# cs2mosa/Heterogeneous-MOE-for-Diffusion-models

Measured on AMD Instinct MI355X. Metric: denoise-steps/sec (fwd+bwd) on 4x32x32 latents, higher is better.
Workload: dtype bf16

## Files before the change

heterogeneous-moe-for-diffusion-models_amd/csrc/bwd6.hip:

```cpp
#include "common.h"
#include "conv_args.h"
#include "conv6_common.h"
#include "hdmoe.h"
#include "conv6_body.h"
#include "conv7_body.h"
#include "wgrad6_body.h"
#include "wgrad7_body.h"
#include "wgrad8_body.h"
#include "conv6s_body.h"

namespace {

template <int MT, int NT, int TWS, int OT>
__global__ __launch_bounds__(512) void bwd6_kernel(C6Args c, W6Args a3, W6Args a5, int G6, int ibs, int obs) {
  const int b = blockIdx.x;
  if (b < G6) { conv6_body<MT, NT>(c, b, G6); return; }
  int r = b - G6;
  const int bx = r % ibs; r /= ibs;
  const int by = r % obs;
  const int z = r / obs;
  if (z < a3.chunks) wgrad6_body<3, TWS, OT, false>(a3, bx, by, z);
  else wgrad6_body<5, TWS, OT, false>(a5, bx, by, z - a3.chunks);
}

template <int MT, int NT, int TWS, int OT>
void launch_bwd6(const C6Plan& cp, const W6DualPlan& wp, hipStream_t stream) {
  static unsigned long long attr = 0;
  if (hdmoe_first_on_device(attr)) { (void)hipFuncSetAttribute((const void*)bwd6_kernel<MT, NT, TWS, OT>, hipFuncAttributeMaxDynamicSharedMemorySize, 160 * 1024); }
  const size_t lds = cp.lds > wp.lds ? cp.lds : wp.lds;
  const unsigned grid = cp.G + (unsigned)(wp.ibs * wp.obs * (wp.c[0].chunks + wp.c[1].chunks));
  hipLaunchKernelGGL((bwd6_kernel<MT, NT, TWS, OT>), dim3(grid), dim3(512), lds, stream, cp.a, wp.c[0], wp.c[1], (int)cp.G, wp.ibs, wp.obs);
}

template <int CO, int KMASK, int TWS, int OT>
__global__ __launch_bounds__(512) void bwd7_kernel(C7Args c, W6Args a3, W6Args a5, int G7, int ibs, int obs) {
  const int b = blockIdx.x;
  if (b < G7) { conv7_body<CO, KMASK, TWS == 4>(c, b, G7); return; }
  int r = b - G7;
  if (TWS == 5 && OT == 0) {
    const int nbx3 = a3.Cin / (32 * a3.icw), nby3 = a3.Cout / (32 * a3.ocw), n3 = nbx3 * nby3 * a3.chunks;
    if (r < n3) {
      const int bx = r % nbx3; r /= nbx3;
      const int by = r % nby3, z = r / nby3, pairs = a3.icw * a3.ocw;
      if (pairs == 0) wgrad7_body<3>(a3, bx, by, z);
      else if (pairs == 4) wgrad8_body3<4, 8>(a3, bx, by, z);
      else if (pairs == 2) wgrad8_body3<2, 8>(a3, bx, by, z);
      else wgrad8_body3<2, 16>(a3, bx, by, z);
      return;
    }
    r -= n3;
    const int bx = r % ibs; r /= ibs;
    wgrad7_body<5>(a5, bx, r % obs, r / obs);
  } else if (OT > 0) {
    const int bx = r % ibs; r /= ibs;
    const int by = r % obs;
    const int z = r / obs;
    if (z < a3.chunks) wgrad6_body<3, TWS, OT == 0 ? 1 : OT, false>(a3, bx, by, z);
    else wgrad6_body<5, TWS, OT == 0 ? 1 : OT, false>(a5, bx, by, z - a3.chunks);
  }
}

template <int CO, int KMASK, int TWS, int OT>
void launch_bwd7(const C7Plan& cp, const W6DualPlan& wp, hipStream_t stream) {
  static unsigned long long attr = 0;
  if (hdmoe_first_on_device(attr)) { (void)hipFuncSetAttribute((const void*)bwd7_kernel<CO, KMASK, TWS, OT>, hipFuncAttributeMaxDynamicSharedMemorySize, 160 * 1024); }
  const size_t lds = cp.lds > wp.lds ? cp.lds : wp.lds;
  const int obs = OT == 0 ? wp.c[0].Cout / 32 : wp.obs;
  unsigned nw = (unsigned)(wp.ibs * obs * (wp.c[0].chunks + wp.c[1].chunks));
  if (OT == 0) nw = (unsigned)((wp.c[0].Cin / (32 * wp.c[0].icw)) * (wp.c[0].Cout / (32 * wp.c[0].ocw)) * wp.c[0].chunks + wp.ibs * obs * wp.c[1].chunks);
  hipLaunchKernelGGL((bwd7_kernel<CO, KMASK, TWS, OT>), dim3(cp.G + nw), dim3(512), lds, stream, cp.a, wp.c[0], wp.c[1], (int)cp.G, wp.ibs, obs);
}

template <int NT, int TWS, int OT>
__global__ __launch_bounds__(512) void bwd6s_kernel(C6SArgs c, W6Args a3, int G6, int ibs, int obs) {
  const int b = blockIdx.x;
  if (b < G6) { conv6s_body<NT>(c, b, G6); return; }
  int r = b - G6;
  const int bx = r % ibs; r /= ibs;
  wgrad6_body<3, TWS, OT, true>(a3, bx, r % obs, r / obs);
}
template <int NT, int TWS, int OT>
void launch_bwd6s(const C6SPlan& cp, const W6DualPlan& wp, hipStream_t stream) {
  static unsigned long long attr = 0;
  if (hdmoe_first_on_device(attr)) { (void)hipFuncSetAttribute((const void*)bwd6s_kernel<NT, TWS, OT>, hipFuncAttributeMaxDynamicSharedMemorySize, 160 * 1024); }
  const size_t lds = cp.lds > wp.lds ? cp.lds : wp.lds;
  const unsigned grid = cp.G + (unsigned)(wp.ibs * wp.obs * wp.c[0].chunks);
  hipLaunchKernelGGL((bwd6s_kernel<NT, TWS, OT>), dim3(grid), dim3(512), lds, stream, cp.sa, wp.c[0], (int)cp.G, wp.ibs, wp.obs);
}

}

extern "C" {

int hdmoe_conv_bwd6s(const void* x, const void* dy, const void* wd, void* dx, float* const* G, const int* seg, int ngroups, long wd_stride,
                     long wd_plane, int N, int H, int W, int Cin, int Cout, const int* kh, const int* kw, const int* pt, const int* pl,
                     float alpha, void* ws, long ws_bytes, const float* in_scale, const float* in_shift, int in_relu, int hi_only, hipStream_t stream) {
  if (!dx || !wd || ngroups < 1 || ngroups > HDMOE_MAX_GROUPS || Cout % 16) return 1;
  W6DualPlan wp;
  if (wgrad6_plan_split(x, dy, G, seg, ngroups, N, H, W, Cin, Cout, kh, kw, pt, pl, ws, ws_bytes, wp)) return 1;
  if ((in_scale == nullptr) != (in_shift == nullptr) || (in_scale && (ngroups != 1 || seg))) return HDMOE_EINVAL;
  wp.c[0].in_scale = in_scale; wp.c[0].in_shift = in_shift; wp.c[0].in_relu = in_relu;
  wp.c[0].hi_only = hi_only ? 1 : 0;
  const ConvArgs c = conv_dgrad_args(dy, wd, dx, seg, ngroups, wd_stride, N, H, W, Cin, Cout, kh, kw, pt, pl, alpha);
  C6SPlan cp;
  if (conv6s_plan(c, wd_plane, nullptr, cp)) return 1;
  cp.sa.nprod = hi_only ? 1 : 3;
  hdmoe_count_selection(HDMOE_SEL_BWD6S);
  conv_pick<2, 1>(cp.NT, [&](auto Nt) { conv_pick<5, 4>(wp.TWS, [&](auto Tws) { conv_pick<2, 1>(wp.OT, [&](auto Ot) {
    launch_bwd6s<decltype(Nt)::value, decltype(Tws)::value, decltype(Ot)::value>(cp, wp, stream);
  }); }); });
  return hdmoe_launch_status();
}

int hdmoe_conv_bwd6(const void* x, const void* dy, const void* wd, void* dx, float* const* G, const int* seg, int ngroups, long wd_stride,
                    int N, int H, int W, int Cin, int Cout, const int* kh, const int* kw, const int* pt, const int* pl, float alpha,
                    void* ws, long ws_bytes, int dtype, hipStream_t stream) {
  if (dtype != HDMOE_BF16 || !dx || !wd || ngroups < 1 || ngroups > HDMOE_MAX_GROUPS || Cout % 16) return 1;
  W6DualPlan wp;
  if (wgrad6_plan_dual(x, dy, G, seg, ngroups, N, H, W, Cin, Cout, kh, kw, pt, pl, ws, ws_bytes, dtype, wp)) return 1;
  const ConvArgs c = conv_dgrad_args(dy, wd, dx, seg, ngroups, wd_stride, N, H, W, Cin, Cout, kh, kw, pt, pl, alpha);
  {
    C7Plan cp7;
    if (!conv7_plan(c, dtype, cp7) && cp7.kmask == 3 && (cp7.w16 != 0) == (wp.TWS == 4)) {
      if (wp.TWS == 5) {
        hdmoe_count_selection(HDMOE_SEL_BWD7_32);
        if (wp.c[0].chunks) {
          hdmoe_count_selection(HDMOE_SEL_BWD7_32_WGRAD8);
          hdmoe_count_selection(wp.c[0].icw == 2 ? (wp.c[0].ocw == 2 ? HDMOE_SEL_WGRAD8_C22 : HDMOE_SEL_WGRAD8_C21)
                                                 : (wp.c[0].ocw == 2 ? HDMOE_SEL_WGRAD8_C12 : HDMOE_SEL_WGRAD8_C11));
        }
        if (wp.c[1].chunks) hdmoe_count_selection(HDMOE_SEL_BWD7_32_WGRAD7);
      } else {
        hdmoe_count_selection(wp.OT == 2 ? HDMOE_SEL_BWD7_16_OT2 : HDMOE_SEL_BWD7_16_OT1);
      }
      conv_pick<2, 1>(cp7.CO, [&](auto Co) {
        if (wp.TWS == 5) launch_bwd7<decltype(Co)::value, 3, 5, 0>(cp7, wp, stream);
        else conv_pick<2, 1>(wp.OT, [&](auto Ot) { launch_bwd7<decltype(Co)::value, 3, 4, decltype(Ot)::value>(cp7, wp, stream); });
      });
      return hdmoe_launch_status();
    }
  }
  C6Plan cp;
  if (conv6_plan(c, dtype, cp)) return 1;
  hdmoe_count_selection(HDMOE_SEL_BWD6);
  conv_pick<2, 1>(cp.MT, [&](auto M) { conv_pick<2, 1>(cp.NT, [&](auto Nt) { conv_pick<5, 4>(wp.TWS, [&](auto Tws) { conv_pick<2, 1>(wp.OT, [&](auto Ot) {
    launch_bwd6<decltype(M)::value, decltype(Nt)::value, decltype(Tws)::value, decltype(Ot)::value>(cp, wp, stream);
  }); }); }); });
  return hdmoe_launch_status();
}

}
```

heterogeneous-moe-for-diffusion-models_amd/csrc/wgrad8_body.h:

```cpp
#pragma once
#include "common.h"
#include "wgrad6_body.h"

namespace {

DEVI bool w8_slot(const W6Args& a, const int zslot, int& n0, int& n1) {
  int gi = 0, chunk = zslot, row0 = 0, units = 0;
  for (; gi < a.ngr; ++gi) {
    const int g = a.groups[gi];
    row0 = a.seg ? __builtin_amdgcn_readfirstlane(a.seg[g]) : 0;
    units = ((a.seg ? __builtin_amdgcn_readfirstlane(a.seg[g + 1]) : a.N) - row0) * a.tpi;
    const int nch = (units + a.upw - 1) / a.upw;
    if (chunk < nch) break;
    chunk -= nch;
  }
  if (gi == a.ngr) return false;
  const int t0 = chunk * a.upw, t1 = min(units, t0 + a.upw);
  n0 = row0 + t0 / 4; n1 = row0 + (t1 + 3) / 4;
  return true;
}

template <int NACC, typename TapOf, typename Store>
DEVI void w8_reduce(unsigned char* lds, const f32x16 (&acc)[NACC], const int NGR, const int wave, const int lane, const int tid, TapOf tap_of, Store store) {
  float* red = reinterpret_cast<float*>(lds);
  const int NP = 8 / NGR;
#pragma unroll
  for (int j0 = 0; j0 < NACC; j0 += 4) {
    const int nr = NACC - j0 < 4 ? NACC - j0 : 4;
    asm volatile("s_waitcnt lgkmcnt(0)\n\ts_barrier" ::: "memory");
#pragma unroll
    for (int jj = 0; jj < 4; ++jj)
      if (jj < nr) {
#pragma unroll
        for (int reg = 0; reg < 16; ++reg) red[((wave * 4 + jj) * 16 + reg) * 64 + lane] = acc[j0 + jj][reg];
      }
    asm volatile("s_waitcnt lgkmcnt(0)\n\ts_barrier" ::: "memory");
    const int ntask = NGR * nr * 256;
    for (int task = tid; task < ntask; task += 512) {
      const int e4 = task & 255, gj = task >> 8, jj = gj % nr, g = gj / nr;
      f32x4 s = (f32x4)(0.f);
      for (int k = 0; k < NP; ++k) s += *reinterpret_cast<const f32x4*>(red + (((g + NGR * k) * 4 + jj) * 1024 + e4 * 4));
      const int el = e4 * 4, reg = el >> 6, ln = el & 63;
      store(g, tap_of(g, j0 + jj), acc_row(reg, ln), ln & 31, s);
    }
  }
}

template <int RPW, int RU>
DEVI void wgrad8_body3(const W6Args& a, const int bx, const int by, const int zslot) {
#if __HIP_DEVICE_COMPILE__
  constexpr int Q = 2;
  constexpr int XROWS = RU + 2, XROWB = 35 * 64, XB = XROWS * XROWB + 3 * 64, DYB = RU * 2048, UPI = 32 / RU;
  extern __shared__ __attribute__((aligned(1024))) unsigned char lds[];
  const int tid = threadIdx.x, lane = tid & 63;
  const int wave = __builtin_amdgcn_readfirstlane(tid >> 6);
  const unsigned lds0 = lds_addr_of(lds);
  const int IC = a.icw, OC = a.ocw, NGR = IC * OC, NP = 8 / NGR;
  const int STAGE = IC * XB + OC * DYB;
  const int i0 = bx * 32 * IC, o0 = by * 32 * OC;
  int nstamp = 0;
  auto stamp = [&](int tag) {
    if (a.stamps && bx == 0 && by == 0 && zslot == 0 && lane == 0 && nstamp < 63) {
      a.stamps[512 + wave * 64 + nstamp] = ((unsigned long long)tag << 56) | (__builtin_amdgcn_s_memtime() & 0x00FFFFFFFFFFFFFFull);
      ++nstamp;
    }
  };
  stamp(1);
  int n0, n1;
  if (!w8_slot(a, zslot, n0, n1)) return;
  const int U = UPI * (n1 - n0);
  const __amdgpu_buffer_rsrc_t rx = __builtin_amdgcn_make_buffer_rsrc(const_cast<void*>(a.x), 0, a.xbytes, 0x00020000);
  const __amdgpu_buffer_rsrc_t rdy = __builtin_amdgcn_make_buffer_rsrc(const_cast<void*>(a.dy), 0, a.dybytes, 0x00020000);

  for (int i = tid; i < 2 * IC * (XROWS + 1) * 12; i += 512) {
    const int til = i / ((XROWS + 1) * 12), k = i % ((XROWS + 1) * 12);
    const int off = (til / IC) * STAGE + (til % IC) * XB + (k / 12) * XROWB + (k % 12) * 16;
    *reinterpret_cast<uint4*>(lds + off) = make_uint4(0, 0, 0, 0);
  }

  const int NXP = IC * XROWS * 2, NPC = NXP + OC * RU * 2;
  const unsigned xl = (unsigned)((lane >> 2) * a.Cin * 2 + (lane & 3) * 16), dyl = (unsigned)((lane >> 2) * a.Cout * 2 + (lane & 3) * 16);
  auto issue_piece = [&](int u, int sb, int k) {
    const int pc = wave + 8 * k;
    if (pc >= NPC) return;
    const int n = n0 + u / UPI, r0 = (u % UPI) * RU;
    if (pc < NXP) {
      const int icp = pc >= XROWS * 2 ? 1 : 0, rem = pc - icp * XROWS * 2, j = rem >> 1, half = rem & 1, row = r0 - 1 + j;
      const bool ok = (unsigned)row < 32u;
      const int so = ((n * 32 + row) * 32 + half * 16) * a.Cin * 2 + (i0 + icp * 32) * 2;
      __builtin_amdgcn_raw_ptr_buffer_load_lds(rx, (lptr_t)(lds + sb + icp * XB + j * XROWB + (3 + half * 16) * 64), 16, ok ? xl : 0xFFFFFFFFu, ok ? so : 0, 0, 0);
    } else {
      const int d = pc - NXP, ocp = d >= RU * 2 ? 1 : 0, rem = d - ocp * RU * 2, j = rem >> 1, half = rem & 1;
      const int so = ((n * 32 + r0 + j) * 32 + half * 16) * a.Cout * 2 + (o0 + ocp * 32) * 2;
      __builtin_amdgcn_raw_ptr_buffer_load_lds(rdy, (lptr_t)(lds + sb + IC * XB + ocp * DYB + j * 2048 + half * 1024), 16, dyl, so, 0, 0);
    }
  };
  constexpr int NPIECE = 10;

  const int h = lane >> 5, cb = (lane >> 4) & 1, q = (lane & 15) >> 2, p4 = lane & 3;
  const int lbase = (8 * h + q) * 64 + cb * 32 + p4 * 8;
  const int grp = wave % NGR, pp = wave / NGR, ic = grp % IC, oc = grp / IC;
  const int xoff = ic * XB + lbase + pp * RPW * XROWB + Q * 64, dyoff = IC * XB + oc * DYB + lbase + pp * RPW * 2048;

  f32x16 acc[9];
#pragma unroll
  for (int t = 0; t < 9; ++t) acc[t] = (f32x16)(0.f);

  stamp(2);
#pragma unroll
  for (int k = 0; k < NPIECE; ++k) issue_piece(0, 0, k);
  stamp(3);
  for (int u = 0; u < U; ++u) {
    stamp(4);
    asm volatile("s_waitcnt vmcnt(0) lgkmcnt(0)\n\ts_barrier" ::: "memory");
    stamp(5);
    const int sb = (u & 1) * STAGE;
    const bool more = u + 1 < U;
    const int xb = sb + xoff, dyb = sb + dyoff;
    hd_s16x4 dl[2][RPW], dh[2][RPW], xl_[2][RPW + 2], xh_[2][RPW + 2];
#pragma unroll
    for (int rr = 0; rr < RPW; ++rr) lds_tr2_issue(dl[0][rr], dh[0][rr], lds0 + dyb + rr * 2048, lds0 + dyb + rr * 2048 + 256);
#pragma unroll
    for (int j = 0; j < RPW + 2; ++j) lds_tr2_issue(xl_[0][j], xh_[0][j], lds0 + xb + j * XROWB, lds0 + xb + j * XROWB + 256);
    bf16x8 fdy[RPW];
#pragma unroll
    for (int c = 0; c < 6; ++c) {
      const int hh = c / 3, kx = c % 3;
      lds_tr_wait();
      bf16x8 fx[RPW + 2];
#pragma unroll
      for (int j = 0; j < RPW + 2; ++j) fx[j] = lds_tr2_take(xl_[c & 1][j], xh_[c & 1][j]);
      if (kx == 0) {
#pragma unroll
        for (int rr = 0; rr < RPW; ++rr) fdy[rr] = lds_tr2_take(dl[hh][rr], dh[hh][rr]);
      }
      if (c + 1 < 6) {
        const int h2 = (c + 1) / 3, k2 = (c + 1) % 3;
#pragma unroll
        for (int j = 0; j < RPW + 2; ++j) {
          const unsigned ad = lds0 + xb + j * XROWB + h2 * 1024 + k2 * 64;
          lds_tr2_issue(xl_[(c + 1) & 1][j], xh_[(c + 1) & 1][j], ad, ad + 256);
        }
        if (c == 1) {
#pragma unroll
          for (int rr = 0; rr < RPW; ++rr) lds_tr2_issue(dl[1][rr], dh[1][rr], lds0 + dyb + rr * 2048 + 1024, lds0 + dyb + rr * 2048 + 1024 + 256);
        }
      }
      if (more && c < 5) { issue_piece(u + 1, STAGE - sb, 2 * c); issue_piece(u + 1, STAGE - sb, 2 * c + 1); }
#pragma unroll
      for (int j = 0; j < RPW + 2; ++j) {
#pragma unroll
        for (int ky = 0; ky < 3; ++ky) {
          const int rr = j - ky;
          if (rr >= 0 && rr < RPW) acc[ky * 3 + kx] = __builtin_amdgcn_mfma_f32_32x32x16_bf16(fdy[rr], fx[j], acc[ky * 3 + kx], 0, 0, 0);
        }
      }
    }
  }
  stamp(6);
  float* Pw = a.ws + (long)zslot * a.ws_item;
  w8_reduce<9>(lds, acc, NGR, wave, lane, tid,
               [](int, int j) { return j; },
               [&](int g, int tap, int o, int i, f32x4 s) {
                 *reinterpret_cast<f32x4*>(Pw + ((long)tap * a.Cout + o0 + (g / IC) * 32 + o) * a.Cin + i0 + (g % IC) * 32 + i) = s;
               });
  stamp(7);
#endif
}

}
```

Baseline: 80.48.

## Add wgrad8 5x5 weight-gradient body and use it in bwd7 fused path

Replaces the wgrad7 5x5 weight-gradient path in the fused bwd7 kernel with a new wgrad8_body5. The new body stages x rows and dy rows into double-buffered LDS through direct buffer-to-LDS loads and uses transposed LDS reads feeding 32x32x16 bf16 MFMAs. Work is split across 8 waves as 4 tap-column groups by 2 row halves, and the extra taps are assigned unevenly through a remapping in the reduction. The aim is better data reuse and overlap of loads with MFMA work for 5x5 weight gradients. The price is a more complex uneven schedule, since wave group 3 handles extra taps.

```diff
diff --git a/heterogeneous-moe-for-diffusion-models_amd/csrc/bwd6.hip b/heterogeneous-moe-for-diffusion-models_amd/csrc/bwd6.hip
--- a/heterogeneous-moe-for-diffusion-models_amd/csrc/bwd6.hip
+++ b/heterogeneous-moe-for-diffusion-models_amd/csrc/bwd6.hip
@@ -50,7 +50,7 @@
     }
     r -= n3;
     const int bx = r % ibs; r /= ibs;
-    wgrad7_body<5>(a5, bx, r % obs, r / obs);
+    wgrad8_body5(a5, bx, r % obs, r / obs);
   } else if (OT > 0) {
     const int bx = r % ibs; r /= ibs;
     const int by = r % obs;
diff --git a/heterogeneous-moe-for-diffusion-models_amd/csrc/wgrad8_body.h b/heterogeneous-moe-for-diffusion-models_amd/csrc/wgrad8_body.h
--- a/heterogeneous-moe-for-diffusion-models_amd/csrc/wgrad8_body.h
+++ b/heterogeneous-moe-for-diffusion-models_amd/csrc/wgrad8_body.h
@@ -168,4 +168,138 @@
 #endif
 }
 
-}
+DEVI void wgrad8_body5(const W6Args& a, const int bx, const int by, const int zslot) {
+#if __HIP_DEVICE_COMPILE__
+  constexpr int XROWS = 20, XROWB = 35 * 64, XB = XROWS * XROWB + 3 * 64, DYB = 16 * 2048, STAGE = XB + DYB;
+  constexpr int NXP = XROWS * 2, NPC = NXP + 32;
+  extern __shared__ __attribute__((aligned(1024))) unsigned char lds[];
+  const int tid = threadIdx.x, lane = tid & 63;
+  const int wave = __builtin_amdgcn_readfirstlane(tid >> 6);
+  const unsigned lds0 = lds_addr_of(lds);
+  const int i0 = bx * 32, o0 = by * 32;
+  int nstamp = 0;
+  auto stamp = [&](int tag) {
+    if (a.stamps && bx == 0 && by == 0 && zslot == 0 && lane == 0 && nstamp < 63) {
+      a.stamps[1024 + wave * 64 + nstamp] = ((unsigned long long)tag << 56) | (__builtin_amdgcn_s_memtime() & 0x00FFFFFFFFFFFFFFull);
+      ++nstamp;
+    }
+  };
+  stamp(1);
+  int n0, n1;
+  if (!w8_slot(a, zslot, n0, n1)) return;
+  const int U = 2 * (n1 - n0);
+  const __amdgpu_buffer_rsrc_t rx = __builtin_amdgcn_make_buffer_rsrc(const_cast<void*>(a.x), 0, a.xbytes, 0x00020000);
+  const __amdgpu_buffer_rsrc_t rdy = __builtin_amdgcn_make_buffer_rsrc(const_cast<void*>(a.dy), 0, a.dybytes, 0x00020000);
+
+  for (int i = tid; i < (XROWS + 1) * 12; i += 512) {
+    const int off = (i / 12) * XROWB + (i % 12) * 16;
+    *reinterpret_cast<uint4*>(lds + off) = make_uint4(0, 0, 0, 0);
+    *reinterpret_cast<uint4*>(lds + STAGE + off) = make_uint4(0, 0, 0, 0);
+  }
+
+  const unsigned xl = (unsigned)((lane >> 2) * a.Cin * 2 + (lane & 3) * 16), dyl = (unsigned)((lane >> 2) * a.Cout * 2 + (lane & 3) * 16);
+  auto issue_piece = [&](int u, int sb, int k) {
+    const int pc = wave + 8 * k;
+    if (pc >= NPC) return;
+    const int n = n0 + (u >> 1), r0 = (u & 1) * 16;
+    if (pc < NXP) {
+      const int j = pc >> 1, half = pc & 1, row = r0 - 2 + j;
+      const bool ok = (unsigned)row < 32u;
+      const int so = ((n * 32 + row) * 32 + half * 16) * a.Cin * 2 + i0 * 2;
+      __builtin_amdgcn_raw_ptr_buffer_load_lds(rx, (lptr_t)(lds + sb + j * XROWB + (3 + half * 16) * 64), 16, ok ? xl : 0xFFFFFFFFu, ok ? so : 0, 0, 0);
+    } else {
+      const int d = pc - NXP, j = d >> 1, half = d & 1;
+      const int so = ((n * 32 + r0 + j) * 32 + half * 16) * a.Cout * 2 + o0 * 2;
+      __builtin_amdgcn_raw_ptr_buffer_load_lds(rdy, (lptr_t)(lds + sb + XB + j * 2048 + half * 1024), 16, dyl, so, 0, 0);
+    }
+  };
+  constexpr int NPIECE = 9;
+
+  const int h = lane >> 5, cb = (lane >> 4) & 1, q = (lane & 15) >> 2, p4 = lane & 3;
+  const int lbase = (8 * h + q) * 64 + cb * 32 + p4 * 8;
+  const int tg = wave & 3, pp = wave >> 2;
+  const bool two = tg == 3;
+  const int xown = lbase + pp * 8 * XROWB + (tg + 1) * 64;
+  const int xex1 = lbase + (pp * 8 + tg) * XROWB + 5 * 64;
+  const int xex2 = lbase + (pp * 8 + 4) * XROWB + 5 * 64;
+  const int dyoff = XB + lbase + pp * 8 * 2048;
+
+  f32x16 acc[7];
+#pragma unroll
+  for (int t = 0; t < 7; ++t) acc[t] = (f32x16)(0.f);
+
+  stamp(2);
+  if (U > 0) {
+#pragma unroll
+    for (int k = 0; k < NPIECE; ++k) issue_piece(0, 0, k);
+  }
+  stamp(3);
+  for (int u = 0; u < U; ++u) {
+    stamp(4);
+    asm volatile("s_waitcnt vmcnt(0) lgkmcnt(0)\n\ts_barrier" ::: "memory");
+    stamp(5);
+    const int sb = (u & 1) * STAGE;
+    const bool more = u + 1 < U;
+    const unsigned dyb = lds0 + sb + dyoff;
+    hd_s16x4 dl[8], dh[8], xl_[2][4], xh_[2][4];
+    auto request = [&](int s) {
+      const int hh = s / 7, b = s % 7;
+      const int base = b < 3 ? xown + 4 * b * XROWB : (b < 5 ? xex1 + 4 * (b - 3) * XROWB : xex2 + 4 * (b - 5) * XROWB);
+#pragma unroll
+      for (int i = 0; i < 4; ++i) {
+        const unsigned ad = lds0 + sb + base + i * XROWB + hh * 1024;
+        lds_tr2_issue(xl_[s & 1][i], xh_[s & 1][i], ad, ad + 256);
+      }
+    };
+#pragma unroll
+    for (int rr = 0; rr < 8; ++rr) lds_tr2_issue(dl[rr], dh[rr], dyb + rr * 2048, dyb + rr * 2048 + 256);
+    request(0);
+    bf16x8 fdy[8];
+#pragma unroll
+    for (int s = 0; s < 14; ++s) {
+      const int hh = s / 7, b = s % 7;
+      if (b >= 5 && !two) continue;
+      if (s == 7) {
+#pragma unroll
+        for (int rr = 0; rr < 8; ++rr) lds_tr2_issue(dl[rr], dh[rr], dyb + rr * 2048 + 1024, dyb + rr * 2048 + 1024 + 256);
+      }
+      lds_tr_wait();
+      bf16x8 fx[4];
+#pragma unroll
+      for (int i = 0; i < 4; ++i) fx[i] = lds_tr2_take(xl_[s & 1][i], xh_[s & 1][i]);
+      if (b == 0) {
+#pragma unroll
+        for (int rr = 0; rr < 8; ++rr) fdy[rr] = lds_tr2_take(dl[rr], dh[rr]);
+      }
+      if (b < 4 || b == 5) request(s + 1);
+      else if (b == 4) { if (two) request(s + 1); else if (hh == 0) request(7); }
+      else if (hh == 0) request(7);
+      if (more && b < 5) issue_piece(u + 1, STAGE - sb, hh * 5 + b);
+      if (b < 3) {
+#pragma unroll
+        for (int i = 0; i < 4; ++i) {
+#pragma unroll
+          for (int ky = 0; ky < 5; ++ky) {
+            const int rr = 4 * b + i - ky;
+            if (rr >= 0 && rr < 8) acc[ky] = __builtin_amdgcn_mfma_f32_32x32x16_bf16(fdy[rr], fx[i], acc[ky], 0, 0, 0);
+          }
+        }
+      } else {
+        const int t = b < 5 ? 5 : 6, r4 = 4 * ((b - 3) & 1);
+#pragma unroll
+        for (int i = 0; i < 4; ++i) acc[t] = __builtin_amdgcn_mfma_f32_32x32x16_bf16(fdy[r4 + i], fx[i], acc[t], 0, 0, 0);
+      }
+    }
+  }
+  stamp(6);
+  float* Pw = a.ws + (long)zslot * a.ws_item;
+  w8_reduce<7>(lds, acc, 4, wave, lane, tid,
+               [](int g, int j) { return j < 5 ? j * 5 + g : (j == 5 ? (g < 3 ? g * 5 + 4 : 19) : (g == 3 ? 24 : -1)); },
+               [&](int, int tap, int o, int i, f32x4 s) {
+                 if (tap >= 0) *reinterpret_cast<f32x4*>(Pw + ((long)tap * a.Cout + o0 + o) * a.Cin + i0 + i) = s;
+               });
+  stamp(7);
+#endif
+}
+
+}
```

Measured after the change: 80.86, median of 6. Within noise of the previous version (+0.5%).
